# dyollb/segmantic

Measured on AMD Instinct MI355X. Metric: 3D UNet train voxels/s on 128^3 bf16, higher is better.
Workload: dtype bf16

## Files before the change

### include/segmi.h

```cpp
#ifndef SEGMI_H_
#define SEGMI_H_

#include <stddef.h>
#include <stdint.h>

#ifdef __cplusplus
extern "C" {
#endif

#define SEGMI_VERSION 1

enum { SEGMI_F32 = 0, SEGMI_BF16 = 1, SEGMI_F16 = 2 };
enum { SEGMI_OK = 0, SEGMI_EINVAL = -1, SEGMI_EUNSUPPORTED = -2, SEGMI_ELAUNCH = -3,
       SEGMI_EDATA = -4  };

typedef struct segmi_act {
  void* data;
  int32_t n, d, h, w;
  int32_t c;
  int32_t ld;
} segmi_act;

int segmi_version(void);
const char* segmi_last_error(void);
// ... 45 lines not shown
  const segmi_act* x;
  const float* mean;
  const float* invstd;
  const float* gamma;
  const float* beta;
  const float* prelu_alpha;
  float* partials;
  const segmi_bn_bwd_fin* fin;
} segmi_bn_bwd_sums;
int segmi_conv3d_bn_bwd_sums_ok(int dtype, const segmi_act* in, const segmi_act* out, int ksize,
                                int stride);
const char* segmi_conv3d_fwd_kernel_name(int dtype, const segmi_act* in, const segmi_act* out,
                                         int ksize, int stride);
int segmi_conv3d_in_affine_ok(int dtype, const segmi_act* in, const segmi_act* out, int ksize,
                              int stride);
int segmi_conv3d_fwd(int dtype, const segmi_act* in, const segmi_act* out, const void* packed,
                     const float* w_src, int w_kind, const float* bias,
                     const float* prelu_alpha, const segmi_act* residual,
                     float* stats_partials, int ksize, int stride, const segmi_in_affine* in_tf,
                     const segmi_bn_bwd_sums* bn_bwd ,
                     const segmi_bn_fin* stats_fin , void* stream);
int segmi_dectop_ok(int dtype, const segmi_act* in, const segmi_act* out);
int segmi_dectop_fwd(int dtype, const segmi_act* in, const segmi_act* out, const void* up_frag,
                     const float* up_bias, const float* up_alpha,
                     int up_alpha_in_unit_range ,
                     const void* conv_packed, const float* conv_bias, void* stream);
typedef struct segmi_windows {
  int32_t count;
  int32_t row_stride;
  int64_t plane_stride;
// ... 29 lines not shown
int segmi_wgrad_cus(int cus);
int segmi_bias_grad(int dtype, const segmi_act* dy, float* db, void* workspace, void* stream);

int segmi_bn_stats_rows(const segmi_act* x);
int segmi_bn_stats(int dtype, const segmi_act* x, float* stats_partials, void* stream);
int segmi_bn_finalize(const float* stats_partials, int rows, int c, double count,
                      const float* gamma, const float* beta, float* running_mean,
                      float* running_var, float momentum, float eps, float* mean,
                      float* invstd, float* scale, float* shift, void* stream);
int segmi_bn_eval_affine(int c, const float* gamma, const float* beta,
                         const float* running_mean, const float* running_var, float eps,
                         float* scale, float* shift, void* stream);
int segmi_bn_act_fwd(int dtype, const segmi_act* x, const segmi_act* y, const float* scale,
                     const float* shift, const float* prelu_alpha, const segmi_act* residual,
                     float dropout_p, uint32_t dropout_seed, void* stream);
int segmi_bn_act_bwd_rows(const segmi_act* x);
int segmi_bn_act_bwd_reduce(int dtype, const segmi_act* dy, const segmi_act* x,
                            const float* mean, const float* invstd, const float* gamma,
                            const float* beta, const float* prelu_alpha, float* red_partials,
                            float dropout_p, uint32_t dropout_seed,
                            const segmi_bn_bwd_fin* fin , void* stream);
int segmi_bn_act_bwd_finalize(const float* red_partials, int rows, int c, double count,
                              const float* gamma, const float* invstd, float* dgamma,
                              float* dbeta, float* dalpha, float* coef, void* stream);
int segmi_bn_act_bwd_fused_ok(int dtype, const segmi_act* dy, const segmi_act* x, const segmi_act* dx);
int segmi_bn_act_bwd_fused_rows(const segmi_act* x);
int segmi_bn_act_bwd_fused_wgs(int dtype, const segmi_act* x, int max_wgs);
int segmi_bn_act_bwd_fused(int dtype, const segmi_act* dy, const segmi_act* x, const segmi_act* dx,
                           const float* mean, const float* invstd, const float* gamma, const float* beta,
                           const float* prelu_alpha, float* red_partials, const segmi_bn_bwd_fin* fin,
// ... 332 lines not shown
```

### segmantic_amd/_lib.py

```python
from __future__ import annotations

import ctypes as C
import os
from pathlib import Path

import torch

SEGMI_F32 = 0
SEGMI_BF16 = 1
SEGMI_F16 = 2

_LIB_PATH = Path(__file__).resolve().parent / "csrc" / "libsegmi.so"


class Act(C.Structure):

    _fields_ = [("data", C.c_void_p), ("n", C.c_int32), ("d", C.c_int32), ("h", C.c_int32),
                ("w", C.c_int32), ("c", C.c_int32), ("ld", C.c_int32)]


class WpackDesc(C.Structure):

    _fields_ = [("w_src", C.c_void_p), ("scale", C.c_void_p), ("packed", C.c_void_p),
                ("kind", C.c_int32), ("cin_k", C.c_int32), ("cout_k", C.c_int32),
# ... 43 lines not shown
_i = C.c_int
_i64 = C.c_int64
_f = C.c_float
_d = C.c_double

SIGNATURES = {
    "segmi_version": (_i, []),
    "segmi_last_error": (C.c_char_p, []),
    "segmi_stream_create_cumask": (_i, [_i, C.POINTER(C.c_void_p)]),
    "segmi_stream_destroy": (_i, [_P]),
    "segmi_wpack_bytes": (_i64, [_i, _i, _i, _i, _i]),
    "segmi_wpack": (_i, [_i, _i, _P, _P, _i, _i, _i, _P, _P]),
    "segmi_wpack_batch": (_i, [_i, C.POINTER(WpackDesc), _i, _P, _i, _P]),
    "segmi_conv3d_stats_rows": (_i, [_i, _AP, _AP, _i, _i]),
    "segmi_conv3d_in_affine_ok": (_i, [_i, _AP, _AP, _i, _i]),
    "segmi_conv3d_fwd_kernel_name": (C.c_char_p, [_i, _AP, _AP, _i, _i]),
    "segmi_conv3d_split_act_ok": (_i, [_i, _AP, _AP, _i, _i]),
    "segmi_conv3d_fwd_split_act": (_i, [_i, _AP, _AP, _P, _P, _P, _i, _i, _i, _P, _P, C.POINTER(BnFin), _P]),
    "segmi_conv3d_fwd": (_i, [_i, _AP, _AP, _P, _P, _i, _P, _P, _AP, _P, _i, _i, C.POINTER(InAffine),
                              C.POINTER(BnBwdSums), C.POINTER(BnFin), _P]),
    "segmi_conv3d_bn_bwd_sums_ok": (_i, [_i, _AP, _AP, _i, _i]),
    "segmi_dectop_ok": (_i, [_i, _AP, _AP]),
    "segmi_dectop_fwd": (_i, [_i, _AP, _AP, _P, _P, _P, _i, _P, _P, _P]),
    "segmi_conv3d_pair_ok": (_i, [_i, _AP, _AP, _AP]),
    "segmi_conv3d_fwd_pair": (_i, [_i, _AP, _AP, _P, _P, _P, _P, _AP, _P, _P, _i, C.POINTER(BnFin),
                                   C.POINTER(Windows), _P]),
    "segmi_convT3d_stats_rows": (_i, [_i, _AP, _AP]),
    "segmi_convT3d_fwd": (_i, [_i, _AP, _AP, _P, _P, _P, _P, _AP, _P, C.POINTER(BnFin), _P]),
    "segmi_conv3d_wgrad_workspace": (_i64, [_i, _AP, _AP, _i, _i, _i]),
    "segmi_conv3d_wgrad": (_i, [_i, _AP, _AP, _P, _P, _i, _i, _P, C.POINTER(InAffine), _i, _P]),
    "segmi_bias_grad": (_i, [_i, _AP, _P, _P, _P]),
    "segmi_bn_stats_rows": (_i, [_AP]),
    "segmi_bn_stats": (_i, [_i, _AP, _P, _P]),
    "segmi_bn_finalize": (_i, [_P, _i, _i, _d, _P, _P, _P, _P, _f, _f, _P, _P, _P, _P, _P]),
    "segmi_bn_eval_affine": (_i, [_i, _P, _P, _P, _P, _f, _P, _P, _P]),
    "segmi_bn_act_fwd": (_i, [_i, _AP, _AP, _P, _P, _P, _AP, _f, C.c_uint32, _P]),
    "segmi_bn_act_bwd_rows": (_i, [_AP]),
    "segmi_bn_act_bwd_reduce": (_i, [_i, _AP, _AP, _P, _P, _P, _P, _P, _P, _f, C.c_uint32,
                                     C.POINTER(BnBwdFin), _P]),
    "segmi_bn_act_bwd_finalize": (_i, [_P, _i, _i, _d, _P, _P, _P, _P, _P, _P, _P]),
    "segmi_bn_act_bwd_fused_ok": (_i, [_i, _AP, _AP, _AP]),
    "segmi_bn_act_bwd_fused_rows": (_i, [_AP]),
    "segmi_bn_act_bwd_fused": (_i, [_i, _AP, _AP, _AP, _P, _P, _P, _P, _P, _P, C.POINTER(BnBwdFin), _i, _P]),
    "segmi_bn_act_bwd_fused_wgs": (_i, [_i, _AP, _i]),
    "segmi_fused_timeouts": (C.c_uint, [_i]),
    "segmi_fused_test_hook": (_i, [C.c_uint, _i]),
    "segmi_bn_act_bwd_apply": (_i, [_i, _AP, _AP, _AP, _P, _P, _P, _P, _P, _P, _f, C.c_uint32, _P]),
    "segmi_bn_act_bwd_apply_conv_ok": (_i, [_i, _AP, _AP, _AP, _AP]),
    "segmi_bn_act_bwd_apply_conv": (_i, [_i, _AP, _AP, _AP, _P, _P, _P, _P, _P, _P, _AP, _P, _P]),
    "segmi_wgrad_cus": (_i, [_i]),
    "segmi_add": (_i, [_i, _AP, _AP, _AP, _P]),
# ... 153 lines not shown
```

### segmantic_amd/csrc/conv.hip

```cpp
#include "conv_fwd_impl.h"
#include "conv_ks_impl.h"
#include "convt_ps_impl.h"
#include "conv_bnbwd_impl.h"

namespace segmi {

int conv_s2_bnbwd_bf16(const ConvBnBwdParams& p, hipStream_t st);
int conv_s2_bnbwd_f16(const ConvBnBwdParams& p, hipStream_t st);

int conv_mfma_f32(const ConvParams& p, const ConvPlan& pl, int ksize, int stride, hipStream_t st);
int conv_mfma_bf16(const ConvParams& p, const ConvPlan& pl, int ksize, int stride, hipStream_t st);
int conv_mfma_f16(const ConvParams& p, const ConvPlan& pl, int ksize, int stride, hipStream_t st);
int convt_mfma_f32(const ConvTParams& p, const ConvTPlan& pl, hipStream_t st);
int convt_mfma_bf16(const ConvTParams& p, const ConvTPlan& pl, hipStream_t st);
int convt_mfma_f16(const ConvTParams& p, const ConvTPlan& pl, hipStream_t st);
static inline int conv_mfma_dt(int dtype, const ConvParams& p, const ConvPlan& pl, int ksize, int stride, hipStream_t st) {
  if (dtype == SEGMI_F32) return conv_mfma_f32(p, pl, ksize, stride, st);
  if (dtype == SEGMI_F16) return conv_mfma_f16(p, pl, ksize, stride, st);
  SEGMI_CHECK_ARG(dtype == SEGMI_BF16, "conv3d: unknown dtype code %d", dtype);
  return conv_mfma_bf16(p, pl, ksize, stride, st);
}
static inline int convt_mfma_dt(int dtype, const ConvTParams& p, const ConvTPlan& pl, hipStream_t st) {
  if (dtype == SEGMI_F32) return convt_mfma_f32(p, pl, st);
  if (dtype == SEGMI_F16) return convt_mfma_f16(p, pl, st);
// ... 245 lines not shown
}

const char* segmi_conv3d_fwd_kernel_name(int dtype, const segmi_act* in, const segmi_act* out,
                                         int ksize, int stride) {
  static thread_local char buf[96];
  if (!act_ok(in) || !act_ok(out)) return "invalid";
  return conv_plan_name(query_plan(dtype, in, out, ksize, stride), dtype, ksize, stride, buf, sizeof buf);
}

int segmi_conv3d_in_affine_ok(int dtype, const segmi_act* in, const segmi_act* out, int ksize,
                              int stride) {
  if (!act_ok(in) || !act_ok(out) || !dtype_h16(dtype) || !mfma_ok(in->c, out->c)) return 0;
  return query_plan(dtype, in, out, ksize, stride).in_affine ? 1 : 0;
}

int segmi_conv3d_bn_bwd_sums_ok(int dtype, const segmi_act* in, const segmi_act* out, int ksize,
                                int stride) {
  if (!act_ok(in) || !act_ok(out) || !dtype_h16(dtype)) return 0;
  return query_plan(dtype, in, out, ksize, stride).bn_bwd_sums ? 1 : 0;
}

int segmi_bn_act_bwd_apply_conv_ok(int dtype, const segmi_act* dy, const segmi_act* x, const segmi_act* dx,
                                   const segmi_act* out) {
  if (!dtype_h16(dtype) || !act_ok(dy) || !act_ok(x) || !act_ok(dx) || !act_ok(out)) return 0;
  const segmi_act* a3[3] = {dy, x, dx};
  for (const segmi_act* a : a3) {
    if (a->n != dy->n || a->d != dy->d || a->h != dy->h || a->w != dy->w || a->c != 16) return 0;
    if (a->ld % 8 != 0 || ((uintptr_t)a->data % 16) != 0) return 0;
  }
  if (out->n != dy->n || out->d != out_extent(dy->d, 3, 2) || out->h != out_extent(dy->h, 3, 2) ||
// ... 28 lines not shown
                     const float* prelu_alpha, const segmi_act* residual,
                     float* stats_partials, int ksize, int stride, const segmi_in_affine* in_tf,
                     const segmi_bn_bwd_sums* bn_bwd, const segmi_bn_fin* stats_fin, void* stream) {
  SEGMI_CHECK_ARG(!stats_fin || (stats_partials && bn_fin_ok(stats_fin)),
                  "conv3d: stats_fin needs stats_partials and its output pointers");
  if (bn_bwd && bn_bwd->fin)
    SEGMI_CHECK_ARG(bn_bwd->fin->count > 0 && bn_bwd->fin->coef, "conv3d: bn_bwd->fin needs count and coef");
  if (bn_bwd)
    SEGMI_CHECK_ARG(bn_bwd->x && act_ok(bn_bwd->x) && bn_bwd->mean && bn_bwd->invstd && bn_bwd->partials &&
                        segmi_conv3d_bn_bwd_sums_ok(dtype, in, out, ksize, stride) && !prelu_alpha &&
                        !stats_partials && bn_bwd->x->n == out->n && bn_bwd->x->d == out->d &&
                        bn_bwd->x->h == out->h && bn_bwd->x->w == out->w && bn_bwd->x->c == out->c &&
                        bn_bwd->x->ld % 4 == 0 && ((uintptr_t)bn_bwd->x->data % 8) == 0,
                    "conv3d: this launch cannot take BatchNorm-backward sums (ask segmi_conv3d_bn_bwd_sums_ok)");
  if (in_tf)
    SEGMI_CHECK_ARG(in_tf->scale && in_tf->shift && segmi_conv3d_in_affine_ok(dtype, in, out, ksize, stride),
                    "conv3d: this layer cannot take an input transform (ask segmi_conv3d_in_affine_ok)");
  SEGMI_CHECK_ARG(dtype_ok(dtype), "conv3d: bad dtype %d", dtype);
  SEGMI_CHECK_ARG(act_ok(in) && act_ok(out), "conv3d: bad activation view");
  SEGMI_CHECK_ARG((ksize == 1 || ksize == 3) && (stride == 1 || stride == 2),
                  "conv3d: unsupported ksize/stride %d/%d", ksize, stride);
  SEGMI_CHECK_ARG(!(ksize == 1 && stride != 1), "conv3d: k1 is stride 1 only");
  SEGMI_CHECK_ARG(in->n == out->n && out->d == out_extent(in->d, ksize, stride) &&
                      out->h == out_extent(in->h, ksize, stride) &&
                      out->w == out_extent(in->w, ksize, stride),
                  "conv3d: output extent [%d,%d,%d,%d] does not match input [%d,%d,%d,%d] k%d s%d",
                  out->n, out->d, out->h, out->w, in->n, in->d, in->h, in->w, ksize, stride);
  SEGMI_CHECK_ARG(!residual || residual_matches(residual, out), "conv3d: residual shape mismatch");
  hipStream_t st = (hipStream_t)stream;
  const ConvPlan pl = conv_plan(dtype, in, out, ksize, stride, residual ? residual->ld : 0, bn_bwd ? bn_bwd->x->ld : 0);
  if (mfma_ok(in->c, out->c)) {
    SEGMI_CHECK_ARG(packed, "conv3d: MFMA path needs a fragment-packed weight (segmi_wpack)");
// ... 80 lines not shown
```

### segmantic_amd/csrc/conv_ks_impl.h

```cpp
#pragma once
#include "conv_fwd_impl.h"

namespace segmi {

template <typename T, int CK, int KS, int S, int NT, int TD, int TH, int TW>
__global__ __launch_bounds__(256) void conv_fwd_ks_kernel(ConvParams p) {
  using G = ConvGeom<T, CK, KS, S, TD, TH, TW>;
  static_assert(G::SPT == 4, "k-split kernel: one k-step per tap");
  static_assert(G::NVT == 8, "k-split kernel: 8 voxel tiles per workgroup");
  constexpr int NSW = (G::NSTEP + 3) / 4;
  extern __shared__ __attribute__((aligned(16))) char smem[];
  const int tid = threadIdx.x, lane = tid & 63;
  const int wave = __builtin_amdgcn_readfirstlane(tid >> 6);
  const int g = lane >> 4, r = lane & 15;

  int t = blockIdx.x;
  const int txi = t % p.tx; t /= p.tx;
  const int tyi = t % p.ty; t /= p.ty;
  const int tzi = t % p.tz;
  const int n = t / p.tz;
  const int oz0 = tzi * TD, oy0 = tyi * TH, ox0 = txi * TW;
  const int iz0 = oz0 * S - G::PAD, iy0 = oy0 * S - G::PAD, ix0 = ox0 * S - G::PAD;
  const int nt0 = blockIdx.y * NT;

// ... 10 lines not shown
    const int x = idx % TW, y = (idx / TW) % TH, z = idx / (TW * TH);
    vaddr[i] = ((z * S * G::HH + y * S) * G::HW + x * S) * G::ROWB + g * 16;
  }
  int tapoff[NSW];
#pragma unroll
  for (int si = 0; si < NSW; ++si) {
    int tap = wave + 4 * si;
    if (tap > G::NTAPS - 1) tap = G::NTAPS - 1;
    tapoff[si] = (((tap / (KS * KS)) * G::HH + (tap / KS) % KS) * G::HW + tap % KS) * G::ROWB;
  }

  constexpr int NCH = G::HD * G::HH * G::HW * G::CPR;
  constexpr int NLD = (NCH + 255) / 256;
  const char* inb = (const char*)p.in;
  frag_t stg[NLD];
  auto fetch = [&](int c) {
#pragma unroll
    for (int k = 0; k < NLD; ++k) {
      const int i = tid + 256 * k;
      const int v = i / G::CPR, ch = i % G::CPR;
      const int hx = v % G::HW, hy = (v / G::HW) % G::HH, hz = v / (G::HW * G::HH);
      const int z = iz0 + hz, y = iy0 + hy, x = ix0 + hx;
      stg[k] = frag_t{0u, 0u, 0u, 0u};
      if (i < NCH && (unsigned)z < (unsigned)p.Di && (unsigned)y < (unsigned)p.Hi &&
          (unsigned)x < (unsigned)p.Wi) {
        const int64_t e = ((((int64_t)n * p.Di + z) * p.Hi + y) * p.Wi + x) * p.ldi + c * CK;
        stg[k] = *reinterpret_cast<const frag_t*>(inb + e * (int64_t)sizeof(T) + ch * 16);
      }
    }
  };
  const char* wb0 = (const char*)p.wfrag + (int64_t)nt0 * 1024 + lane * 16;
  frag_t wcur[NSW][NT], wnxt[NSW][NT];
  auto fetch_w = [&](int c, frag_t (&dst)[NSW][NT]) {
#pragma unroll
    for (int si = 0; si < NSW; ++si) {
      int s = wave + 4 * si;
      if (s > G::NSTEP - 1) s = G::NSTEP - 1;
#pragma unroll
      for (int j = 0; j < NT; ++j)
        dst[si][j] = *reinterpret_cast<const frag_t*>(
            wb0 + (((int64_t)c * G::NSTEP + s) * p.ntiles_total + j) * 1024);
    }
  };
  fetch(0);
  fetch_w(0, wcur);
  for (int c = 0; c < p.nchunks; ++c) {
    if (c > 0) __syncthreads();
#pragma unroll
    for (int k = 0; k < NLD; ++k) {
      const int i = tid + 256 * k;
      if (i < NCH) *reinterpret_cast<frag_t*>(smem + (i / G::CPR) * G::ROWB + (i % G::CPR) * 16) = stg[k];
    }
    __syncthreads();
    if (c + 1 < p.nchunks) {
      fetch(c + 1);
      fetch_w(c + 1, wnxt);
    }
#pragma unroll
    for (int si = 0; si < NSW; ++si) {
      const int s = wave + 4 * si;
      if (s < G::NSTEP) {
#pragma unroll
        for (int i = 0; i < 8; ++i) {
          const frag_t a = *reinterpret_cast<const frag_t*>(smem + vaddr[i] + tapoff[si]);
#pragma unroll
          for (int j = 0; j < NT; ++j) acc[i][j] = mma16<T>(wcur[si][j], a, acc[i][j]);
// ... 43 lines not shown
  T* outp = (T*)p.out;
  const T* resp = (const T*)p.res;
  f32x4 resv[2][NT];
  if (resp) {
#pragma unroll
    for (int ii = 0; ii < 2; ++ii) {
      const int idx = (wave * 2 + ii) * 16 + r;
      const int oz = oz0 + idx / (TW * TH), oy = oy0 + (idx / TW) % TH, ox = ox0 + idx % TW;
      const bool valid = oz < p.Do && oy < p.Ho && ox < p.Wo;
      const int64_t vox = (((int64_t)n * p.Do + oz) * p.Ho + oy) * p.Wo + ox;
#pragma unroll
      for (int j = 0; j < NT; ++j)
        resv[ii][j] = valid ? load4<T>(resp + vox * p.ldr + (nt0 + j) * 16 + 4 * g)
                            : f32x4{0.f, 0.f, 0.f, 0.f};
    }
#pragma unroll
    for (int ii = 0; ii < 2; ++ii)
#pragma unroll
      for (int j = 0; j < NT; ++j) touch_v(resv[ii][j]);
  }
#pragma unroll
  for (int j = 0; j < NT; ++j) touch_v(bias4[j]);
#pragma unroll
  for (int k = 0; k < NLD; ++k) touch_v(stg[k]);
#pragma unroll
  for (int ii = 0; ii < 2; ++ii) {
    const int idx = (wave * 2 + ii) * 16 + r;
    const int oz = oz0 + idx / (TW * TH), oy = oy0 + (idx / TW) % TH, ox = ox0 + idx % TW;
    const bool valid = oz < p.Do && oy < p.Ho && ox < p.Wo;
    const int64_t vox = (((int64_t)n * p.Do + oz) * p.Ho + oy) * p.Wo + ox;
// ... 29 lines not shown
          rs[(wave * 2 + 1) * NT * 16 + j * 16 + 4 * g + e] = b;
        }
      }
    __syncthreads();
    if (tid < 2 * NT * 16) {
      const int which = tid / (NT * 16), ch = tid % (NT * 16);
      float sacc = 0.f;
#pragma unroll
      for (int w = 0; w < 4; ++w) sacc += rs[(w * 2 + which) * NT * 16 + ch];
      fin_store(&p.stats[((int64_t)blockIdx.x * 2 + which) * p.Cout + nt0 * 16 + ch], sacc);
    }
    fin_tail_run<BnFin, 256, offsetof(ConvParams, ft), offsetof(ConvParams, bfin)>(p.stats, smem);
  }
}

template <typename T, int CK, int KS, int S, int NT, int TD, int TH, int TW>
static int launch_conv_ks_cfg(ConvParams p, const ConvPlan& pl, hipStream_t st) {
  using G = ConvGeom<T, CK, KS, S, TD, TH, TW>;
  p.tz = pl.tz; p.ty = pl.ty; p.tx = pl.tx;
  SEGMI_CHECK_ARG(TD == pl.td && TH == pl.th && TW == pl.tw && pl.grid_x > 0 && (int64_t)p.N * p.tz * p.ty * p.tx == pl.grid_x,
                  "conv3d: too many tiles, or the k-split kernel's grid is not the planned one");
  dim3 grid((unsigned)pl.grid_x, (unsigned)(p.Cout / (16 * NT)));
  constexpr int red = 4 * 8 * NT * 64 * 16;
  constexpr int lds0 = G::LDS_BYTES > red ? G::LDS_BYTES : red;
  p.fin_on = p.fin_on && p.stats;
  const size_t lds = fin_tail_arm(p, grid, 256, 2 * p.Cout, lds0);
  return launch_wg256<conv_fwd_ks_kernel<T, CK, KS, S, NT, TD, TH, TW>>(grid, lds, lds > 64 * 1024, st,
                                                                       "conv3d_fwd(mfma, k-split)", p);
}

template <typename T, int CK>
static int launch_conv_ks(const ConvParams& p, const ConvPlan& pl, hipStream_t st) {
#define KS_CASE(NT, WIDE)                                                          \
  case NT * 32 + conv_ks_tile_shape(WIDE).tw: {                                    \
    constexpr Tile3 t = conv_ks_tile_shape(WIDE);                                  \
    return launch_conv_ks_cfg<T, CK, 3, 1, NT, t.td, t.th, t.tw>(p, pl, st);       \
  }
  switch (pl.nt * 32 + pl.tw) { KS_CASE(2, true) KS_CASE(2, false) KS_CASE(1, true) KS_CASE(1, false) }
#undef KS_CASE
  SEGMI_UNSUPPORTED("conv3d: no k-split kernel of %d output tiles per workgroup", pl.nt);
}

}
```

### segmantic_amd/csrc/conv_plan.h

```cpp
#pragma once
#include "common.h"

namespace segmi {

int bn_stats_rows_for(const segmi_act* x);
int wgrad_cus(int cus);

constexpr int kFillWgs = 512;
constexpr int kRingMinWgs = 256;
constexpr int64_t kOffsetLimit = 1ll << 31;
constexpr bool wide_row(int w) { return w > 8; }

struct Tile3 { int td, th, tw; };
constexpr Tile3 conv_tile_shape(int stride, bool wide) {
  return stride == 1 ? (wide ? Tile3{4, 8, 16} : Tile3{4, 4, 8}) : (wide ? Tile3{2, 4, 16} : Tile3{2, 4, 8});
}
constexpr Tile3 conv_ks_tile_shape(bool wide) { return wide ? Tile3{2, 4, 16} : Tile3{4, 4, 8}; }
constexpr Tile3 kRingTile{4, 8, 16}, kSmallFwdTile{4, 8, 16};
constexpr Tile3 convt_tile_shape(bool wide) { return wide ? Tile3{2, 2, 16} : Tile3{2, 4, 8}; }
constexpr Tile3 kConvTPsTile{2, 2, 16};
constexpr int kCtPsMaxTiles = 16;
constexpr int kCtPsTargetWgs = 1024;

static inline int64_t tile_count(const Tile3& t, int n, int d, int h, int w, int* tz, int* ty, int* tx) {
// ... 9 lines not shown
static inline bool mfma_ok(int cin, int cout) { return cin % 16 == 0 && cout % 16 == 0; }
static inline bool conv_small_ok(int cin, int cout, int ksize) {
  return ksize == 3 && cin >= 1 && cin <= 4 && (cout == 16 || cout == 32);
}

enum ConvFamily { kConvRing3, kConvRing2, kConvKSplit, kConvTile, kConvSmallCin, kConvDirect };

struct ConvPlan {
  int family;
  int ck;
  int nt;
  int td, th, tw;
  int tz, ty, tx, zsplit;
  int grid_x, grid_y;
  bool in_affine;
  bool bn_bwd_sums;
  bool split_act;
};

static inline int conv_ring_zsplit(int dtype, int cin, int ksize, int stride, const segmi_act* out) {
  if (!(ksize == 3 && stride == 1 && cin == pick_ck(dtype, cin) && wide_row(out->w) && dtype_h16(dtype))) return 0;
  if ((int64_t)(out->d + 8) * out->h * out->w * (4 * cin) * 2 >= kOffsetLimit) return 0;
  const int columns = out->n * cdiv(out->h, kRingTile.th) * cdiv(out->w, kRingTile.tw);
  const int steps = cdiv(out->d, kRingTile.td);
  int zs = kFillWgs / columns;
  if (zs < 1) zs = 1;
  if (zs > steps / 4) zs = steps / 4;
  return zs < 1 || columns * zs < kRingMinWgs ? 0 : zs;
}
static inline bool conv_ring3_shape_ok(const segmi_act* in, const segmi_act* out, int ldr, int ldbx) {
  if (in->c != 16 || out->c % 16 != 0) return false;
  const int64_t isample = (int64_t)(in->d + 8) * in->h * in->w, osample = (int64_t)(out->d + 4) * out->h * out->w;
  return isample * in->ld * 2 < kOffsetLimit && osample * out->ld * 2 < kOffsetLimit &&
         osample * (ldr > 0 ? ldr : 1) * 2 < kOffsetLimit && osample * (ldbx > 0 ? ldbx : 1) * 2 < kOffsetLimit &&
         ((uintptr_t)in->data % 16) == 0 && in->ld % 8 == 0 &&
         ((uintptr_t)out->data % 16) == 0 && out->ld % 8 == 0;
}
static inline bool conv_ks_ok(int dtype, int cin, int ksize, int stride) {
  const int ck = pick_ck(dtype, cin), spt = ck / (dtype == SEGMI_F32 ? 4 : 8);
  return ksize == 3 && stride == 1 && spt == 4 && cin >= ck;
}

static inline ConvPlan conv_plan(int dtype, const segmi_act* in, const segmi_act* out, int ksize, int stride, int ldr,
                                 int ldbx) {
  ConvPlan pl{};
  const bool wide = wide_row(out->w);
  const int ntiles = out->c / 16;
  pl.ck = pick_ck(dtype, in->c);
  pl.nt = pl.grid_y = 1;
  Tile3 t;
  if (!mfma_ok(in->c, out->c)) {
    pl.family = conv_small_ok(in->c, out->c, ksize) && out->ld % 4 == 0 &&
                ((uintptr_t)out->data % (4 * dtype_size(dtype))) == 0 ? kConvSmallCin : kConvDirect;
    if (pl.family == kConvDirect) { pl.grid_x = bn_stats_rows_for(out); return pl; }
    t = kSmallFwdTile;
// ... 5 lines not shown
    pl.bn_bwd_sums = (in->c == 16 && out->c == 16) || (in->c == 32 && out->c == 32);
  } else if (conv_ks_ok(dtype, in->c, ksize, stride)) {
    pl.family = kConvKSplit;
    t = conv_ks_tile_shape(wide);
  } else {
    pl.family = kConvTile;
    t = conv_tile_shape(stride, wide);
    pl.split_act = ksize == 3 && stride == 2;
  }
  pl.td = t.td; pl.th = t.th; pl.tw = t.tw;
  int64_t wgs = tile_count(t, out->n, pl.zsplit ? t.td : out->d, out->h, out->w, &pl.tz, &pl.ty, &pl.tx);
  if (pl.zsplit) { pl.tz = pl.zsplit; wgs *= pl.zsplit; }
  pl.grid_x = grid_of(wgs);
  if (pl.family == kConvKSplit) {
    if (ntiles % 2 == 0 && wgs * (ntiles / 2) >= kFillWgs) pl.nt = 2;
  } else if (pl.family == kConvTile) {
    pl.nt = ntiles % 4 == 0 ? 4 : (ntiles % 2 == 0 ? 2 : 1);
    while (pl.nt > 1 && wgs * (ntiles / pl.nt) < kFillWgs) pl.nt /= 2;
  }
  pl.grid_y = ntiles / pl.nt;
  return pl;
}

static inline int conv_ring_mode(const ConvPlan& pl, bool sums, bool prelu, bool stats) {
  return pl.bn_bwd_sums && sums && !prelu && !stats ? 4 : (prelu ? 1 : 0) | (stats ? 2 : 0);
}

static inline const char* conv_plan_name(const ConvPlan& pl, int dtype, int ksize, int stride, char* buf, size_t n) {
  const char* dt = dtype_name(dtype);
  switch (pl.family) {
// ... 124 lines not shown
```

### segmantic_amd/csrc/norm_act.hip

```cpp
#include <string.h>

#include <map>
#include <mutex>
#include <tuple>

#include "common.h"
#include "fin_tail.h"

namespace segmi {

static inline int stat_vox(int64_t nvox, int c) {
  const int want = c <= 16 ? 1024 : 512;
  int v = 4096;
  while (v > 64 && nvox / v < want) v >>= 1;
  while (v < 4096 && cdiv64(nvox, v) * 3 * c > 65536) v <<= 1;
  return v;
}
constexpr int kReserveRows = 2 * kFinScratchRows + 1;

int bn_stats_rows_for(const segmi_act* x) {
  return (int)cdiv64(act_voxels(x), stat_vox(act_voxels(x), x->c));
}
int stats_reserve_rows() { return kReserveRows; }

// ... 23 lines not shown
  int64_t nvox;
  int c, ldx, ldy, ldr, ldo, vpw;
  const float* p0; const float* p1; const float* p2; const float* p3; const float* alpha;
  const float* coef;
  float* out_partials;
  int fin_on;
  FinTail ft;
  BnBwdFin bbfin;
  BiasFin biasfin;
  unsigned epoch;
  unsigned poll_limit;
  unsigned* tmo;
  int no_publish;
  unsigned drop_thresh, drop_seed;
  float drop_scale;
};

__device__ __forceinline__ float drop_mult(unsigned seed, int64_t elem, unsigned thresh, float scale) {
  unsigned h = (unsigned)elem * 0x9E3779B1u ^ seed ^ ((unsigned)(elem >> 32) * 0x85EBCA77u);
  h ^= h >> 16; h *= 0x7feb352du; h ^= h >> 15; h *= 0x846ca68bu; h ^= h >> 16;
  return (h >> 8) >= thresh ? scale : 0.f;
}

template <typename T, int VEC>
__global__ __launch_bounds__(256) void bn_stats_kernel(EwParams p) {
  __shared__ float red[256 * 2 * VEC];
  const int cg = p.c / VEC;
  const int vpp = 256 / cg > 0 ? 256 / cg : 1;
  const int tid = threadIdx.x;
  const int my_cg = tid % cg, my_v = tid / cg;
// ... 110 lines not shown
    const int ch = (int)(e - v * cg) * VEC;
    float a[VEC];
    loadv<T, VEC>(x + v * p.ldx + ch, a);
#pragma unroll
    for (int k = 0; k < VEC; ++k) {
      float z = fmaf(a[k], prm[ch + k], prm[p.c + ch + k]);
      if (p.drop_thresh) z *= drop_mult(p.drop_seed, v * p.c + ch + k, p.drop_thresh, p.drop_scale);
      if (has_alpha) z = z > 0.f ? z : alpha * z;
      a[k] = z;
    }
    if (r) {
      float b[VEC];
      loadv<T, VEC>(r + v * p.ldr + ch, b);
#pragma unroll
      for (int k = 0; k < VEC; ++k) a[k] += b[k];
    }
    storev<T, VEC>(o + v * p.ldo + ch, a);
  }
}

template <typename T, int VEC>
__global__ __launch_bounds__(256) void bn_act_bwd_reduce_kernel(EwParams p) {
  __shared__ float red[256 * 3 * VEC];
  const int cg = p.c / VEC;
  const int vpp = 256 / cg > 0 ? 256 / cg : 1;
  const int tid = threadIdx.x;
  const int my_cg = tid % cg, my_v = tid / cg;
  const int64_t v0 = (int64_t)blockIdx.x * p.vpw;
  const int64_t v1 = v0 + p.vpw < p.nvox ? v0 + p.vpw : p.nvox;
  const T* x = (const T*)p.x;
// ... 390 lines not shown
  SEGMI_CHECK_ARG(dtype_ok(dtype), "bn_act_fwd: bad dtype");
  SEGMI_CHECK_ARG(dropout_p >= 0.f && dropout_p < 1.f, "bn_act_fwd: dropout_p must be in [0, 1)");
  SEGMI_CHECK_ARG(act_ok(x) && act_ok(y) && same_shape(x, y), "bn_act_fwd: shape mismatch");
  if (residual) SEGMI_CHECK_ARG(act_ok(residual) && same_shape(x, residual), "bn_act_fwd: residual shape");
  EwParams p{};
  p.drop_thresh = (unsigned)(dropout_p * 16777216.0f); p.drop_seed = dropout_seed;
  p.drop_scale = 1.0f / (1.0f - dropout_p);
  p.x = x->data; p.o = y->data; p.r = residual ? residual->data : nullptr;
  p.nvox = act_voxels(x); p.c = x->c; p.ldx = x->ld; p.ldo = y->ld;
  p.ldr = residual ? residual->ld : 0;
  p.p0 = scale; p.p1 = shift; p.alpha = prelu_alpha;
  const bool v4 = vec4_ok(x, dtype) && vec4_ok(y, dtype) && (!residual || vec4_ok(residual, dtype));
  const int grid = grid_1d(p.nvox * (x->c / (v4 ? 4 : 1)), kEwCap);
  DISPATCH_TV(bn_act_fwd_kernel, dtype, v4, grid, 2 * x->c * sizeof(float), (hipStream_t)stream, p);
  SEGMI_LAUNCH_CHECK("bn_act_fwd");
  return SEGMI_OK;
}

int segmi_add(int dtype, const segmi_act* a, const segmi_act* b, const segmi_act* out,
              void* stream) {
  return segmi_bn_act_fwd(dtype, a, out, nullptr, nullptr, nullptr, b, 0.f, 0u, stream);
}

int segmi_bn_act_bwd_rows(const segmi_act* x) { return x ? bn_stats_rows_for(x) + kReserveRows : 0; }

int segmi_bn_act_bwd_reduce(int dtype, const segmi_act* dy, const segmi_act* x,
                            const float* mean, const float* invstd, const float* gamma,
                            const float* beta, const float* prelu_alpha, float* red_partials,
                            float dropout_p, uint32_t dropout_seed, const segmi_bn_bwd_fin* fin,
                            void* stream) {
// ... 227 lines not shown
```

### segmantic_amd/ops.py

```python
from __future__ import annotations

import ctypes as C
import math
from typing import Optional, Sequence

import numpy as np
import torch

from . import _lib
from ._lib import SEGMI_BF16, SEGMI_F16, SEGMI_F32, Act, BnBwdFin, BnBwdSums, BnFin, InAffine, Windows, check, lib

_DT = {torch.float32: SEGMI_F32, torch.bfloat16: SEGMI_BF16, torch.float16: SEGMI_F16}


def dtype_code(t: torch.Tensor) -> int:
    try:
        return _DT[t.dtype]
    except KeyError:
        raise TypeError(f"unsupported activation dtype {t.dtype} (float32 / bfloat16 / float16 only)")


def _stream() -> int:
    return torch.cuda.current_stream().cuda_stream

# ... 137 lines not shown
        return None
    scale, shift, alpha = in_tf
    for t in (scale, shift):
        if t.dtype != torch.float32 or not t.is_contiguous():
            raise ValueError("in_tf: contiguous float32 scale / shift expected")
    return C.byref(InAffine(_ptr(scale), _ptr(shift), _ptr(alpha)))


def conv3d_fwd_kernel_name(x, y, ksize, stride) -> str:
    ax, ay = act(x), act(y)
    return lib.segmi_conv3d_fwd_kernel_name(dtype_code(x), C.byref(ax), C.byref(ay), ksize, stride).decode()


def conv3d_in_affine_ok(x, y, ksize, stride) -> bool:
    ax, ay = act(x), act(y)
    return bool(lib.segmi_conv3d_in_affine_ok(dtype_code(x), C.byref(ax), C.byref(ay), ksize, stride))


def conv3d_bn_bwd_sums_ok(x, y, ksize, stride) -> bool:
    ax, ay = act(x), act(y)
    return bool(lib.segmi_conv3d_bn_bwd_sums_ok(dtype_code(x), C.byref(ax), C.byref(ay), ksize, stride))


def wgrad_cus(cus: int) -> int:
    return int(lib.segmi_wgrad_cus(int(cus)))


def cu_masked_stream(cus_enabled: int, device=None) -> "torch.cuda.Stream":
    dev = torch.device("cuda", torch.cuda.current_device()) if device is None else torch.device(device)
    h = C.c_void_p()
    with torch.cuda.device(dev):
# ... 123 lines not shown

def bn_finalize(partials, rows, c, count, gamma, beta, running_mean, running_var, momentum,
                eps, mean, invstd, scale, shift) -> None:
    check(lib.segmi_bn_finalize(_ptr(partials), rows, c, float(count), _ptr(gamma), _ptr(beta),
                                _ptr(running_mean), _ptr(running_var), momentum, eps,
                                _ptr(mean), _ptr(invstd), _ptr(scale), _ptr(shift), _stream()),
          "bn_finalize")


def bn_eval_affine(gamma, beta, running_mean, running_var, eps, scale, shift) -> None:
    check(lib.segmi_bn_eval_affine(running_mean.numel(), _ptr(gamma), _ptr(beta),
                                   _ptr(running_mean), _ptr(running_var), eps, _ptr(scale),
                                   _ptr(shift), _stream()), "bn_eval_affine")


def bn_act_fwd(x, y, scale, shift, prelu_alpha=None, residual=None, dropout=(0.0, 0)) -> None:
    ax, ay = act(x), act(y)
    ar = act(residual) if residual is not None else None
    check(lib.segmi_bn_act_fwd(dtype_code(x), C.byref(ax), C.byref(ay), _ptr(scale),
                               _ptr(shift), _ptr(prelu_alpha), _ref(ar), float(dropout[0]),
                               int(dropout[1]) & 0xFFFFFFFF, _stream()),
          "bn_act_fwd")


def bn_act_bwd_rows(x) -> int:
    ax = act(x)
    return int(lib.segmi_bn_act_bwd_rows(C.byref(ax)))


def bn_act_bwd_reduce(dy, x, mean, invstd, gamma, beta, prelu_alpha, partials,
                      dropout=(0.0, 0), fin=None) -> None:
    ady, ax = act(dy), act(x)
    bf = _bn_bwd_fin(fin)
# ... 1640 lines not shown
```

### segmantic_amd/seg/unet.py

```python
from __future__ import annotations

import math
import os
from typing import Dict, List, Optional, Sequence, Tuple

import torch
import torch.nn as nn

from .. import ops
from . import streams

_HALF = (torch.bfloat16, torch.float16)


class _Box(nn.Module):
    """Name-space node: holds children / parameters, computes nothing."""


def _conv_params(cin: int, cout: int, k: int, dims: int, transposed: bool) -> _Box:
    m = _Box()
    shape = ((cin, cout) if transposed else (cout, cin)) + (k,) * dims
    w = torch.empty(shape)
    nn.init.kaiming_uniform_(w, a=math.sqrt(5))
    fan_in = shape[1] * k ** dims
# ... 640 lines not shown
        if not sums_rows:
            part = self._fstat(ops.bn_act_bwd_rows(x_raw), bn.c)
            ops.bn_act_bwd_reduce(dy, x_raw, bn.mean, bn.invstd, bn.gamma, bn.beta, bn.alpha, part,
                                  dropout=bn.drop(), fin=self._bwd_fin(bn, x_raw))
        if (then_conv is not None and self.fuse_apply_conv and self.dropout_p <= 0.0 and then_conv[0].transposed
                and ops.bn_act_bwd_apply_conv_ok(dy, x_raw, dx, then_conv[1])):
            ops.bn_act_bwd_apply_conv(dy, x_raw, dx, bn.mean, bn.invstd, bn.gamma, bn.beta, bn.alpha, bn.coef,
                                      then_conv[1], then_conv[0].dgrad_pack())
            return True
        ops.bn_act_bwd_apply(dy, x_raw, dx, bn.mean, bn.invstd, bn.gamma, bn.beta, bn.alpha,
                             bn.coef, dropout=bn.drop())
        return False

    def _ru_fwd_train(self, ru, x, out, in_tf=None):
        pre = ru["prefix"]
        n, d, h, w = self._down_shape(x.shape, ru["stride"])
        cur = x
        nun = len(ru["units"])
        saved = {"x": x}
        paired = False
        tpair = None
        if ru["res"] is not None:
            rc = ru["res"]
            paired = self._pair_ok(ru, x, out, f"{pre}.r0", (n, d, h, w))
            if not paired and in_tf is None:
                tpair = self._train_pair(ru, x, (n, d, h, w))
            if not paired and tpair is None:
                ops.conv3d_fwd(x, out, rc.fwd_pack(), rc.w, 0, rc.b, rc.k, rc.stride)
            resid = out
        else:
# ... 38 lines not shown
                    cur = a
                continue
            if bn is None:
                self._timed(conv.prefix + ":fwd", ops.conv3d_fwd, cur, out, conv.fwd_pack(), conv.w,
                            0, conv.b, conv.k, conv.stride, residual=resid, in_tf=in_tf)
                saved[f"in{i}"] = cur
                saved[f"tf{i}"] = in_tf
                break
            r = self._buf(f"{pre}.r{i}", (n, d, h, w, conv.cout))
            self._conv_train(conv, cur, r, bn, in_tf=in_tf)
            saved[f"in{i}"] = cur
            saved[f"r{i}"] = r
            saved[f"tf{i}"] = in_tf
            in_tf = None
            if last:
                ops.bn_act_fwd(r, out, bn.scale, bn.shift, bn.alpha, residual=resid, dropout=bn.drop())
            else:
                nconv = ru["units"][i + 1][0]
                if self._tf_ok(r, r, nconv) and nconv.cin == conv.cout and nconv.cout == conv.cout:
                    in_tf = (bn.scale, bn.shift, bn.alpha)
                    cur = r
                else:
                    a = self._buf(f"{pre}.a{i}", (n, d, h, w, conv.cout))
                    ops.bn_act_fwd(r, a, bn.scale, bn.shift, bn.alpha, dropout=bn.drop())
                    cur = a
        self._saved[pre] = saved

    def _ru_bwd(self, ru, dout, dx=None, extra=None, dx_bn=None):
        pre = ru["prefix"]
        sv = self._saved[pre]
        x = sv["x"]
# ... 98 lines not shown
        ru_fwd = self._ru_fwd_train if train else self._ru_fwd_eval
        ru_fwd(lvl["down"], x, down_out)
        if lvl["sub"] is not None:
            self._level_fwd(lvl["sub"], down_out, sub_out, train)
        else:
            ru_fwd(lvl["bottom"], down_out, sub_out)
        up, ubn = lvl["upconv"], lvl["upbn"]
        oshape = (x.shape[0], x.shape[1], x.shape[2], x.shape[3], lvl["outc"])
        if train:
            if id(lvl) in self._carry_lvls:
                self.sync_weights()
            u = self._buf(f"{p}u", oshape)
            self._conv_train(up, cat, u, ubn)
            upru = lvl["upru"]
            conv0, bn0 = upru["units"][0]
            if (bn0 is None and upru["res"] is None and conv0.cin == conv0.cout == lvl["outc"]
                    and self._tf_ok(u, out, conv0)):
                self._saved[p + "up"] = {"cat": cat, "u": u}
                self._ru_fwd_train(upru, u, out, in_tf=(ubn.scale, ubn.shift, ubn.alpha))
            else:
                au = self._buf(f"{p}au.t", oshape)
                ops.bn_act_fwd(u, au, ubn.scale, ubn.shift, ubn.alpha, dropout=ubn.drop())
                self._saved[p + "up"] = {"cat": cat, "u": u}
                self._ru_fwd_train(upru, au, out)
        else:
            sc, sh = ubn.eval_affine()
            upru = lvl["upru"]
            conv0, bn0 = upru["units"][0]
            if (self.fuse_eval_top and lvl["is_top"] and self.dtype in _HALF and bn0 is None
                    and upru["res"] is None and up.cin == 32 and up.cout == 16 and conv0.cin == conv0.cout == 16
                    and ops.dectop_ok(cat, out)):
# ... 238 lines not shown
```

Before: 3.631 billion.

## Fuse upconv BN-PReLU into k-split conv input and residual epilogue

Adds an input-transform (BN affine plus PReLU) variant of the k-split 3x3 conv kernel, applied while staging input tiles into LDS with a halo-validity mask, and a transformed residual path in the epilogue. Adds a bn_act_fwd variant that applies a second affine/PReLU to the residual. Together these let decoder up-residual units with a BN unit take the raw upconv output, skipping a separate materialised bn_act pass and its memory traffic. In exchange the conv uses more LDS and does per-element transform work, and the transform only covers single-tile (nt==1) plans.

```diff
diff --git a/include/segmi.h b/include/segmi.h
--- a/include/segmi.h
+++ b/include/segmi.h
@@ -83,6 +83,8 @@
                                          int ksize, int stride);
 int segmi_conv3d_in_affine_ok(int dtype, const segmi_act* in, const segmi_act* out, int ksize,
                               int stride);
+int segmi_conv3d_in_affine_ks_ok(int dtype, const segmi_act* in, const segmi_act* out, int ksize,
+                                 int stride);
 int segmi_conv3d_fwd(int dtype, const segmi_act* in, const segmi_act* out, const void* packed,
                      const float* w_src, int w_kind, const float* bias,
                      const float* prelu_alpha, const segmi_act* residual,
@@ -142,6 +144,9 @@
 int segmi_bn_act_fwd(int dtype, const segmi_act* x, const segmi_act* y, const float* scale,
                      const float* shift, const float* prelu_alpha, const segmi_act* residual,
                      float dropout_p, uint32_t dropout_seed, void* stream);
+int segmi_bn_act_fwd_res_tf(int dtype, const segmi_act* x, const segmi_act* y, const float* scale,
+                            const float* shift, const float* prelu_alpha, const segmi_act* residual,
+                            const segmi_in_affine* res_tf, void* stream);
 int segmi_bn_act_bwd_rows(const segmi_act* x);
 int segmi_bn_act_bwd_reduce(int dtype, const segmi_act* dy, const segmi_act* x,
                             const float* mean, const float* invstd, const float* gamma,
diff --git a/segmantic_amd/_lib.py b/segmantic_amd/_lib.py
--- a/segmantic_amd/_lib.py
+++ b/segmantic_amd/_lib.py
@@ -81,6 +81,7 @@
     "segmi_wpack_batch": (_i, [_i, C.POINTER(WpackDesc), _i, _P, _i, _P]),
     "segmi_conv3d_stats_rows": (_i, [_i, _AP, _AP, _i, _i]),
     "segmi_conv3d_in_affine_ok": (_i, [_i, _AP, _AP, _i, _i]),
+    "segmi_conv3d_in_affine_ks_ok": (_i, [_i, _AP, _AP, _i, _i]),
     "segmi_conv3d_fwd_kernel_name": (C.c_char_p, [_i, _AP, _AP, _i, _i]),
     "segmi_conv3d_split_act_ok": (_i, [_i, _AP, _AP, _i, _i]),
     "segmi_conv3d_fwd_split_act": (_i, [_i, _AP, _AP, _P, _P, _P, _i, _i, _i, _P, _P, C.POINTER(BnFin), _P]),
@@ -102,6 +103,7 @@
     "segmi_bn_finalize": (_i, [_P, _i, _i, _d, _P, _P, _P, _P, _f, _f, _P, _P, _P, _P, _P]),
     "segmi_bn_eval_affine": (_i, [_i, _P, _P, _P, _P, _f, _P, _P, _P]),
     "segmi_bn_act_fwd": (_i, [_i, _AP, _AP, _P, _P, _P, _AP, _f, C.c_uint32, _P]),
+    "segmi_bn_act_fwd_res_tf": (_i, [_i, _AP, _AP, _P, _P, _P, _AP, C.POINTER(InAffine), _P]),
     "segmi_bn_act_bwd_rows": (_i, [_AP]),
     "segmi_bn_act_bwd_reduce": (_i, [_i, _AP, _AP, _P, _P, _P, _P, _P, _P, _f, C.c_uint32,
                                      C.POINTER(BnBwdFin), _P]),
diff --git a/segmantic_amd/csrc/conv.hip b/segmantic_amd/csrc/conv.hip
--- a/segmantic_amd/csrc/conv.hip
+++ b/segmantic_amd/csrc/conv.hip
@@ -283,6 +283,12 @@
   return query_plan(dtype, in, out, ksize, stride).in_affine ? 1 : 0;
 }
 
+int segmi_conv3d_in_affine_ks_ok(int dtype, const segmi_act* in, const segmi_act* out, int ksize,
+                                 int stride) {
+  if (!act_ok(in) || !act_ok(out) || !dtype_h16(dtype) || !mfma_ok(in->c, out->c)) return 0;
+  return query_plan(dtype, in, out, ksize, stride).in_affine_ks ? 1 : 0;
+}
+
 int segmi_conv3d_bn_bwd_sums_ok(int dtype, const segmi_act* in, const segmi_act* out, int ksize,
                                 int stride) {
   if (!act_ok(in) || !act_ok(out) || !dtype_h16(dtype)) return 0;
@@ -341,8 +347,10 @@
                         bn_bwd->x->ld % 4 == 0 && ((uintptr_t)bn_bwd->x->data % 8) == 0,
                     "conv3d: this launch cannot take BatchNorm-backward sums (ask segmi_conv3d_bn_bwd_sums_ok)");
   if (in_tf)
-    SEGMI_CHECK_ARG(in_tf->scale && in_tf->shift && segmi_conv3d_in_affine_ok(dtype, in, out, ksize, stride),
-                    "conv3d: this layer cannot take an input transform (ask segmi_conv3d_in_affine_ok)");
+    SEGMI_CHECK_ARG(in_tf->scale && in_tf->shift &&
+                        (segmi_conv3d_in_affine_ok(dtype, in, out, ksize, stride) ||
+                         segmi_conv3d_in_affine_ks_ok(dtype, in, out, ksize, stride)),
+                    "conv3d: this layer cannot take an input transform (ask segmi_conv3d_in_affine_ok / _ks_ok)");
   SEGMI_CHECK_ARG(dtype_ok(dtype), "conv3d: bad dtype %d", dtype);
   SEGMI_CHECK_ARG(act_ok(in) && act_ok(out), "conv3d: bad activation view");
   SEGMI_CHECK_ARG((ksize == 1 || ksize == 3) && (stride == 1 || stride == 2),
diff --git a/segmantic_amd/csrc/conv_ks_impl.h b/segmantic_amd/csrc/conv_ks_impl.h
--- a/segmantic_amd/csrc/conv_ks_impl.h
+++ b/segmantic_amd/csrc/conv_ks_impl.h
@@ -3,7 +3,9 @@
 
 namespace segmi {
 
-template <typename T, int CK, int KS, int S, int NT, int TD, int TH, int TW>
+constexpr int kKsTfBytes = (2 * kKsTfChannels + 256 + 4) * (int)sizeof(float);
+
+template <typename T, int CK, int KS, int S, int NT, int TD, int TH, int TW, bool TF = false>
 __global__ __launch_bounds__(256) void conv_fwd_ks_kernel(ConvParams p) {
   using G = ConvGeom<T, CK, KS, S, TD, TH, TW>;
   static_assert(G::SPT == 4, "k-split kernel: one k-step per tap");
@@ -48,6 +50,47 @@
   constexpr int NLD = (NCH + 255) / 256;
   const char* inb = (const char*)p.in;
   frag_t stg[NLD];
+  float* tfs = reinterpret_cast<float*>(smem + G::LDS_BYTES);
+  unsigned* tfm = reinterpret_cast<unsigned*>(tfs + 2 * kKsTfChannels);
+  if constexpr (TF) {
+    static_assert(G::LDS_BYTES % 16 == 0 && NLD <= 32 && 256 % G::CPR == 0 && kKsTfChannels == 256,
+                  "k-split input transform: table / mask layout");
+    tfs[tid] = tid < p.Cin ? p.in_scale[tid] : 1.f;
+    tfs[kKsTfChannels + tid] = tid < p.Cin ? p.in_shift[tid] : 0.f;
+    if (tid == 0) {
+      tfs[2 * kKsTfChannels + 256] = p.in_alpha ? *p.in_alpha : 0.f;
+      tfm[256 + 1] = p.in_alpha ? 1u : 0u;
+    }
+    unsigned inside = 0u;
+#pragma unroll
+    for (int k = 0; k < NLD; ++k) {
+      const int i = tid + 256 * k;
+      const int v = i / G::CPR;
+      const int hx = v % G::HW, hy = (v / G::HW) % G::HH, hz = v / (G::HW * G::HH);
+      if (i < NCH && (unsigned)(iz0 + hz) < (unsigned)p.Di && (unsigned)(iy0 + hy) < (unsigned)p.Hi &&
+          (unsigned)(ix0 + hx) < (unsigned)p.Wi)
+        inside |= 1u << k;
+    }
+    tfm[tid] = inside;
+  }
+  auto commit_tf = [&](int c) {
+    if constexpr (TF) {
+      float sc[8], sh[8];
+      const float* t0 = tfs + c * CK + 8 * (tid % G::CPR);
+#pragma unroll
+      for (int e = 0; e < 8; ++e) { sc[e] = t0[e]; sh[e] = t0[kKsTfChannels + e]; }
+      const unsigned inside = tfm[tid];
+      const float tf_alpha = tfs[2 * kKsTfChannels + 256];
+      const bool tf_act = tfm[256 + 1] != 0u;
+#pragma unroll
+      for (int k = 0; k < NLD; ++k) {
+        const int i = tid + 256 * k;
+        if (i < NCH)
+          *reinterpret_cast<frag_t*>(smem + (i / G::CPR) * G::ROWB + (i % G::CPR) * 16) =
+              (inside >> k) & 1u ? bn_prelu_h8<T>(stg[k], sc, sh, tf_alpha, tf_act) : frag_t{0u, 0u, 0u, 0u};
+      }
+    }
+  };
   auto fetch = [&](int c) {
 #pragma unroll
     for (int k = 0; k < NLD; ++k) {
@@ -78,12 +121,17 @@
   };
   fetch(0);
   fetch_w(0, wcur);
+  if constexpr (TF) __syncthreads();
   for (int c = 0; c < p.nchunks; ++c) {
     if (c > 0) __syncthreads();
-#pragma unroll
-    for (int k = 0; k < NLD; ++k) {
-      const int i = tid + 256 * k;
-      if (i < NCH) *reinterpret_cast<frag_t*>(smem + (i / G::CPR) * G::ROWB + (i % G::CPR) * 16) = stg[k];
+    if constexpr (TF) {
+      commit_tf(c);
+    } else {
+#pragma unroll
+      for (int k = 0; k < NLD; ++k) {
+        const int i = tid + 256 * k;
+        if (i < NCH) *reinterpret_cast<frag_t*>(smem + (i / G::CPR) * G::ROWB + (i % G::CPR) * 16) = stg[k];
+      }
     }
     __syncthreads();
     if (c + 1 < p.nchunks) {
@@ -157,6 +205,30 @@
         resv[ii][j] = valid ? load4<T>(resp + vox * p.ldr + (nt0 + j) * 16 + 4 * g)
                             : f32x4{0.f, 0.f, 0.f, 0.f};
     }
+    if constexpr (TF) {
+      if (p.res == p.in && p.ldr == p.ldi && p.Cin == p.Cout) {
+        const bool tf_act = p.in_alpha != nullptr;
+        const float tf_alpha = tf_act ? *p.in_alpha : 0.f;
+#pragma unroll
+        for (int j = 0; j < NT; ++j) {
+          const int co = (nt0 + j) * 16 + 4 * g;
+          float rsc[4], rsh[4];
+#pragma unroll
+          for (int e = 0; e < 4; ++e) { rsc[e] = p.in_scale[co + e]; rsh[e] = p.in_shift[co + e]; }
+#pragma unroll
+          for (int ii = 0; ii < 2; ++ii) {
+            float z[4];
+#pragma unroll
+            for (int e = 0; e < 4; ++e) {
+              z[e] = fmaf(resv[ii][j][e], rsc[e], rsh[e]);
+              if (tf_act) z[e] = z[e] > 0.f ? z[e] : tf_alpha * z[e];
+            }
+            const unsigned u0 = H16<T>::pack2(z[0], z[1]), u1 = H16<T>::pack2(z[2], z[3]);
+            resv[ii][j] = f32x4{H16<T>::lo(u0), H16<T>::hi(u0), H16<T>::lo(u1), H16<T>::hi(u1)};
+          }
+        }
+      }
+    }
 #pragma unroll
     for (int ii = 0; ii < 2; ++ii)
 #pragma unroll
@@ -216,7 +288,7 @@
   }
 }
 
-template <typename T, int CK, int KS, int S, int NT, int TD, int TH, int TW>
+template <typename T, int CK, int KS, int S, int NT, int TD, int TH, int TW, bool TF>
 static int launch_conv_ks_cfg(ConvParams p, const ConvPlan& pl, hipStream_t st) {
   using G = ConvGeom<T, CK, KS, S, TD, TH, TW>;
   p.tz = pl.tz; p.ty = pl.ty; p.tx = pl.tx;
@@ -224,21 +296,31 @@
                   "conv3d: too many tiles, or the k-split kernel's grid is not the planned one");
   dim3 grid((unsigned)pl.grid_x, (unsigned)(p.Cout / (16 * NT)));
   constexpr int red = 4 * 8 * NT * 64 * 16;
-  constexpr int lds0 = G::LDS_BYTES > red ? G::LDS_BYTES : red;
+  constexpr int stage = G::LDS_BYTES + (TF ? kKsTfBytes : 0);
+  constexpr int lds0 = stage > red ? stage : red;
+  if constexpr (TF) {
+    SEGMI_CHECK_ARG(pl.in_affine_ks && p.Cin <= kKsTfChannels, "conv3d: the k-split plan takes no input transform");
+  }
   p.fin_on = p.fin_on && p.stats;
   const size_t lds = fin_tail_arm(p, grid, 256, 2 * p.Cout, lds0);
-  return launch_wg256<conv_fwd_ks_kernel<T, CK, KS, S, NT, TD, TH, TW>>(grid, lds, lds > 64 * 1024, st,
-                                                                       "conv3d_fwd(mfma, k-split)", p);
+  return launch_wg256<conv_fwd_ks_kernel<T, CK, KS, S, NT, TD, TH, TW, TF>>(grid, lds, lds > 64 * 1024, st,
+                                                                           "conv3d_fwd(mfma, k-split)", p);
 }
 
 template <typename T, int CK>
 static int launch_conv_ks(const ConvParams& p, const ConvPlan& pl, hipStream_t st) {
-#define KS_CASE(NT, WIDE)                                                          \
+#define KS_CASE(NT, WIDE, TF)                                                      \
   case NT * 32 + conv_ks_tile_shape(WIDE).tw: {                                    \
     constexpr Tile3 t = conv_ks_tile_shape(WIDE);                                  \
-    return launch_conv_ks_cfg<T, CK, 3, 1, NT, t.td, t.th, t.tw>(p, pl, st);       \
-  }
-  switch (pl.nt * 32 + pl.tw) { KS_CASE(2, true) KS_CASE(2, false) KS_CASE(1, true) KS_CASE(1, false) }
+    return launch_conv_ks_cfg<T, CK, 3, 1, NT, t.td, t.th, t.tw, TF>(p, pl, st);   \
+  }
+  if (p.in_scale) {
+    if constexpr (sizeof(T) == 2) {
+      switch (pl.nt * 32 + pl.tw) { KS_CASE(1, true, true) KS_CASE(1, false, true) }
+    }
+    SEGMI_UNSUPPORTED("conv3d: no k-split kernel with an input transform for this layer");
+  }
+  switch (pl.nt * 32 + pl.tw) { KS_CASE(2, true, false) KS_CASE(2, false, false) KS_CASE(1, true, false) KS_CASE(1, false, false) }
 #undef KS_CASE
   SEGMI_UNSUPPORTED("conv3d: no k-split kernel of %d output tiles per workgroup", pl.nt);
 }
diff --git a/segmantic_amd/csrc/conv_plan.h b/segmantic_amd/csrc/conv_plan.h
--- a/segmantic_amd/csrc/conv_plan.h
+++ b/segmantic_amd/csrc/conv_plan.h
@@ -47,6 +47,7 @@
   int tz, ty, tx, zsplit;
   int grid_x, grid_y;
   bool in_affine;
+  bool in_affine_ks;
   bool bn_bwd_sums;
   bool split_act;
 };
@@ -72,6 +73,11 @@
 static inline bool conv_ks_ok(int dtype, int cin, int ksize, int stride) {
   const int ck = pick_ck(dtype, cin), spt = ck / (dtype == SEGMI_F32 ? 4 : 8);
   return ksize == 3 && stride == 1 && spt == 4 && cin >= ck;
+}
+constexpr int kKsTfChannels = 256;
+static inline bool conv_ks_in_affine_ok(int dtype, int cin, int nt, bool wide) {
+  (void)wide;
+  return dtype_h16(dtype) && cin <= kKsTfChannels && nt == 1;
 }
 
 static inline ConvPlan conv_plan(int dtype, const segmi_act* in, const segmi_act* out, int ksize, int stride, int ldr,
@@ -107,6 +113,7 @@
   pl.grid_x = grid_of(wgs);
   if (pl.family == kConvKSplit) {
     if (ntiles % 2 == 0 && wgs * (ntiles / 2) >= kFillWgs) pl.nt = 2;
+    pl.in_affine_ks = conv_ks_in_affine_ok(dtype, in->c, pl.nt, wide);
   } else if (pl.family == kConvTile) {
     pl.nt = ntiles % 4 == 0 ? 4 : (ntiles % 2 == 0 ? 2 : 1);
     while (pl.nt > 1 && wgs * (ntiles / pl.nt) < kFillWgs) pl.nt /= 2;
diff --git a/segmantic_amd/csrc/norm_act.hip b/segmantic_amd/csrc/norm_act.hip
--- a/segmantic_amd/csrc/norm_act.hip
+++ b/segmantic_amd/csrc/norm_act.hip
@@ -61,6 +61,7 @@
   int no_publish;
   unsigned drop_thresh, drop_seed;
   float drop_scale;
+  const float* r_alpha;
 };
 
 __device__ __forceinline__ float drop_mult(unsigned seed, int64_t elem, unsigned thresh, float scale) {
@@ -201,6 +202,41 @@
       loadv<T, VEC>(r + v * p.ldr + ch, b);
 #pragma unroll
       for (int k = 0; k < VEC; ++k) a[k] += b[k];
+    }
+    storev<T, VEC>(o + v * p.ldo + ch, a);
+  }
+}
+
+template <typename T, int VEC>
+__global__ __launch_bounds__(256) void bn_act_fwd_res_tf_kernel(EwParams p) {
+  extern __shared__ float prm[];
+  for (int i = threadIdx.x; i < p.c; i += 256) {
+    prm[i] = p.p0 ? p.p0[i] : 1.f;
+    prm[p.c + i] = p.p1 ? p.p1[i] : 0.f;
+    prm[2 * p.c + i] = p.p2[i];
+    prm[3 * p.c + i] = p.p3[i];
+  }
+  __syncthreads();
+  const bool has_alpha = p.alpha != nullptr, has_ralpha = p.r_alpha != nullptr;
+  const float alpha = has_alpha ? *p.alpha : 0.f, ralpha = has_ralpha ? *p.r_alpha : 0.f;
+  const int cg = p.c / VEC;
+  const int64_t total = p.nvox * cg;
+  const T* x = (const T*)p.x;
+  const T* r = (const T*)p.r;
+  T* o = (T*)p.o;
+  for (int64_t e = blockIdx.x * 256ll + threadIdx.x; e < total; e += (int64_t)gridDim.x * 256) {
+    const int64_t v = e / cg;
+    const int ch = (int)(e - v * cg) * VEC;
+    float a[VEC], b[VEC];
+    loadv<T, VEC>(x + v * p.ldx + ch, a);
+    loadv<T, VEC>(r + v * p.ldr + ch, b);
+#pragma unroll
+    for (int k = 0; k < VEC; ++k) {
+      float z = fmaf(a[k], prm[ch + k], prm[p.c + ch + k]);
+      if (has_alpha) z = z > 0.f ? z : alpha * z;
+      float q = fmaf(b[k], prm[2 * p.c + ch + k], prm[3 * p.c + ch + k]);
+      if (has_ralpha) q = q > 0.f ? q : ralpha * q;
+      a[k] = z + H16<T>::lo(H16<T>::pack2(q, 0.f));
     }
     storev<T, VEC>(o + v * p.ldo + ch, a);
   }
@@ -621,6 +657,28 @@
   const int grid = grid_1d(p.nvox * (x->c / (v4 ? 4 : 1)), kEwCap);
   DISPATCH_TV(bn_act_fwd_kernel, dtype, v4, grid, 2 * x->c * sizeof(float), (hipStream_t)stream, p);
   SEGMI_LAUNCH_CHECK("bn_act_fwd");
+  return SEGMI_OK;
+}
+
+int segmi_bn_act_fwd_res_tf(int dtype, const segmi_act* x, const segmi_act* y, const float* scale,
+                            const float* shift, const float* prelu_alpha, const segmi_act* residual,
+                            const segmi_in_affine* res_tf, void* stream) {
+  SEGMI_CHECK_ARG(dtype_h16(dtype), "bn_act_fwd_res_tf: bf16 / fp16 storage only");
+  SEGMI_CHECK_ARG(act_ok(x) && act_ok(y) && same_shape(x, y), "bn_act_fwd_res_tf: shape mismatch");
+  SEGMI_CHECK_ARG(residual && act_ok(residual) && same_shape(x, residual), "bn_act_fwd_res_tf: residual shape");
+  SEGMI_CHECK_ARG(res_tf && res_tf->scale && res_tf->shift, "bn_act_fwd_res_tf: res_tf needs scale and shift");
+  EwParams p{};
+  p.x = x->data; p.o = y->data; p.r = residual->data;
+  p.nvox = act_voxels(x); p.c = x->c; p.ldx = x->ld; p.ldo = y->ld; p.ldr = residual->ld;
+  p.p0 = scale; p.p1 = shift; p.alpha = prelu_alpha;
+  p.p2 = res_tf->scale; p.p3 = res_tf->shift; p.r_alpha = res_tf->prelu_alpha;
+  const bool v4 = vec4_ok(x, dtype) && vec4_ok(y, dtype) && vec4_ok(residual, dtype);
+  const int grid = grid_1d(p.nvox * (x->c / (v4 ? 4 : 1)), kEwCap);
+  const size_t lds = 4 * x->c * sizeof(float);
+  SEGMI_CHECK_ARG(lds <= 64 * 1024, "bn_act_fwd_res_tf: too many channels");
+  if (dtype == SEGMI_BF16) LAUNCH_TV(bf16_t, bn_act_fwd_res_tf_kernel, v4, grid, lds, (hipStream_t)stream, p);
+  else LAUNCH_TV(f16_t, bn_act_fwd_res_tf_kernel, v4, grid, lds, (hipStream_t)stream, p);
+  SEGMI_LAUNCH_CHECK("bn_act_fwd_res_tf");
   return SEGMI_OK;
 }
 
diff --git a/segmantic_amd/ops.py b/segmantic_amd/ops.py
--- a/segmantic_amd/ops.py
+++ b/segmantic_amd/ops.py
@@ -175,7 +175,8 @@
 
 def conv3d_in_affine_ok(x, y, ksize, stride) -> bool:
     ax, ay = act(x), act(y)
-    return bool(lib.segmi_conv3d_in_affine_ok(dtype_code(x), C.byref(ax), C.byref(ay), ksize, stride))
+    args = (dtype_code(x), C.byref(ax), C.byref(ay), ksize, stride)
+    return bool(lib.segmi_conv3d_in_affine_ok(*args) or lib.segmi_conv3d_in_affine_ks_ok(*args))
 
 
 def conv3d_bn_bwd_sums_ok(x, y, ksize, stride) -> bool:
@@ -329,9 +330,16 @@
                                    _ptr(shift), _stream()), "bn_eval_affine")
 
 
-def bn_act_fwd(x, y, scale, shift, prelu_alpha=None, residual=None, dropout=(0.0, 0)) -> None:
+def bn_act_fwd(x, y, scale, shift, prelu_alpha=None, residual=None, dropout=(0.0, 0), residual_tf=None) -> None:
     ax, ay = act(x), act(y)
     ar = act(residual) if residual is not None else None
+    if residual_tf is not None:
+        if residual is None or float(dropout[0]) != 0.0:
+            raise ValueError("bn_act_fwd: residual_tf needs a residual and no dropout")
+        check(lib.segmi_bn_act_fwd_res_tf(dtype_code(x), C.byref(ax), C.byref(ay), _ptr(scale), _ptr(shift),
+                                          _ptr(prelu_alpha), C.byref(ar), _in_affine(residual_tf), _stream()),
+              "bn_act_fwd_res_tf")
+        return
     check(lib.segmi_bn_act_fwd(dtype_code(x), C.byref(ax), C.byref(ay), _ptr(scale),
                                _ptr(shift), _ptr(prelu_alpha), _ref(ar), float(dropout[0]),
                                int(dropout[1]) & 0xFFFFFFFF, _stream()),
diff --git a/segmantic_amd/seg/unet.py b/segmantic_amd/seg/unet.py
--- a/segmantic_amd/seg/unet.py
+++ b/segmantic_amd/seg/unet.py
@@ -678,6 +678,7 @@
 
     def _ru_fwd_train(self, ru, x, out, in_tf=None):
         pre = ru["prefix"]
+        res_tf = in_tf if ru["res"] is None else None
         n, d, h, w = self._down_shape(x.shape, ru["stride"])
         cur = x
         nun = len(ru["units"])
@@ -746,7 +747,8 @@
             saved[f"tf{i}"] = in_tf
             in_tf = None
             if last:
-                ops.bn_act_fwd(r, out, bn.scale, bn.shift, bn.alpha, residual=resid, dropout=bn.drop())
+                ops.bn_act_fwd(r, out, bn.scale, bn.shift, bn.alpha, residual=resid, dropout=bn.drop(),
+                               residual_tf=res_tf)
             else:
                 nconv = ru["units"][i + 1][0]
                 if self._tf_ok(r, r, nconv) and nconv.cin == conv.cout and nconv.cout == conv.cout:
@@ -875,7 +877,7 @@
             self._conv_train(up, cat, u, ubn)
             upru = lvl["upru"]
             conv0, bn0 = upru["units"][0]
-            if (bn0 is None and upru["res"] is None and conv0.cin == conv0.cout == lvl["outc"]
+            if (upru["res"] is None and conv0.cin == conv0.cout == lvl["outc"]
                     and self._tf_ok(u, out, conv0)):
                 self._saved[p + "up"] = {"cat": cat, "u": u}
                 self._ru_fwd_train(upru, u, out, in_tf=(ubn.scale, ubn.shift, ubn.alpha))
```

Result: no change. 3.641 billion, median of 3 (+0.3%).
